# stripe/rainier

Measured on NVIDIA H100. Metric: leapfrog_steps_x_chains_per_sec, higher is better.
Workload: dtype f64

## Files before the change

rainier_b200/csrc/rn_runtime.cpp:

```cpp
#include <dlfcn.h>
#if defined(__x86_64__)
#include <emmintrin.h>
#endif
#include <nvrtc.h>
#include <sys/syscall.h>
#include <unistd.h>

#include <algorithm>
#include <atomic>
#include <cctype>
#include <chrono>
#include <cmath>
#include <cstdio>
#include <cstdlib>
#include <condition_variable>
#include <cstring>
#include <deque>
#include <functional>
#include <map>
#include <memory>
#include <mutex>
#include <sstream>
#include <string>
#include <thread>
// ... 131 lines not shown
}
static unsigned tpc_block_for(size_t chains, unsigned sms) {
  unsigned block = 128u;
  while (block > 32u && chains < (size_t)block * sms * 2) block >>= 1;
  if (const char* e = getenv("RN_BLOCK")) block = std::max(32u, std::min(128u, (unsigned)atoi(e) & ~31u));
  return block;
}
struct Kernel {
  std::string source;
  std::vector<char> cubin;
  CUmodule mod = nullptr;
  CUfunction k_init = nullptr, k_iter = nullptr, k_warmup = nullptr, k_density = nullptr, k_transpose = nullptr, k_pool_reduce = nullptr,
             k_pool_apply = nullptr, k_diag_chain = nullptr, k_diag_reduce = nullptr, k_step_pool = nullptr,
             k_diag_accum = nullptr, k_diag_terms = nullptr,
             k_pool_reduce_dense = nullptr, k_pool_factor = nullptr, k_pool_apply_dense = nullptr;
  const Program* prog = nullptr;
  int backend = 0;
  bool step_pool = false;
  bool mass_pool = false;
  unsigned tpc_block = 0;
  int wpc_smem_doubles = 0;
  int warps_per_cta = 4;
  int wpc_k = 1;
  int tma_stages = 0;
  int tile_doubles = 0;
  bool mma = false;
  int mma_chains = 8;
  unsigned tpc_smem_per_thread = 0;
  unsigned smem_bytes() const {
    size_t d = (size_t)warps_per_cta * wpc_smem_doubles;
    if (tma_stages > 0) d = ((d + 15) & ~(size_t)15) + (size_t)tma_stages * tile_doubles + (size_t)(mma ? 8 : tma_stages);
    return (unsigned)(d * 8);
  }
};

struct rn_model {
  std::recursive_mutex mu;
  std::vector<uint8_t> rir;
  uint32_t n_params = 0, n_inputs = 0;
  bool rir_has_gradient = false;
  int device = -1;
  CUcontext ctx = nullptr;
  CUdeviceptr d_data = 0;
  std::vector<uint64_t> target_base;
  std::vector<int> target_pitch;
  int inlined_targets = 0;
  int64_t inlined_monomials = 0, inlined_rows = 0;
  uint64_t data_doubles = 0;
  std::map<std::pair<bool, bool>, std::unique_ptr<Program>> programs;
  std::map<KernelKey, std::unique_ptr<Kernel>> kernels;
  CUdeviceptr pool[2] = {0, 0};
  CUdeviceptr diag_scratch = 0;
  size_t diag_bytes = 0;
  CUdeviceptr spare_arena = 0;
  size_t spare_arena_bytes = 0;
  CUstream spare_stream = nullptr;
  size_t pool_bytes[2] = {0, 0};
  struct OptKernel {
    std::string source;
    std::vector<char> cubin;
    CUmodule mod = nullptr;
    CUfunction k_lbfgs = nullptr;
    int backend = 0;
    int smem_doubles = 0;
    int starts_per_cta = 1;
    int wpc_k = 1;
  };
  std::map<std::tuple<bool, bool, int, int>, std::unique_ptr<OptKernel>> opt_kernels;
};

static int make_current(const Api* A, rn_model* m) {
  CU(A->cuCtxSetCurrent(m->ctx));
  return RN_OK;
}

static int get_program(rn_model* m, bool adjoint, bool fast, const Program** out) {
  if (!m->rir_has_gradient) adjoint = true;
  auto key = std::make_pair(adjoint, fast);
  auto it = m->programs.find(key);
  if (it == m->programs.end()) {
    std::unique_ptr<Program> P(new Program());
    std::string e = build_program(m->rir.data(), m->rir.size(), adjoint, fast, *P);
    if (!e.empty()) return fail(RN_E_INVALID, e);
    it = m->programs.emplace(key, std::move(P)).first;
  }
  *out = it->second.get();
  return RN_OK;
}

static KernelKey key_for(const rn_model* m, const rn_config* cfg) {
  KernelKey k;
  const int gm = cfg ? cfg->gradient_mode : RN_GRAD_AUTO;
  k.adjoint = (gm == RN_GRAD_ADJOINT) || !m->rir_has_gradient;
  k.fast = cfg && cfg->math_mode == RN_MATH_FAST;
  k.ehmc = cfg && cfg->sampler == RN_SAMPLER_EHMC;
  k.step_pool = cfg && cfg->step_adaptation == RN_ADAPT_POOLED;
  k.mass_pool = cfg && cfg->adaptation == RN_ADAPT_POOLED && cfg->mass_tuner == RN_MASS_DENSE;
  k.mass_max = 0;
  if (cfg) {
    if (cfg->mass_tuner == RN_MASS_DIAGONAL) k.mass_max = 1;
    if (cfg->mass_tuner == RN_MASS_DENSE) k.mass_max = 2;
    if (cfg->mass_tuner == RN_MASS_STATIC) k.mass_max = cfg->static_matrix == RN_MATRIX_DENSE ? 2 : (cfg->static_matrix == RN_MATRIX_DIAGONAL ? 1 : 0);
  }
  int want = cfg ? cfg->backend : RN_BACKEND_AUTO;
  if (const char* e = getenv("RN_BACKEND")) want = atoi(e);
  if (want == RN_BACKEND_AUTO) {
    uint64_t row_work = 0;
    auto it = m->programs.begin();
    if (it != m->programs.end())
      for (const TargetInfo& T : it->second->targets)
        if (T.streamed()) row_work += T.n_rows * (uint64_t)(T.row_fwd.size() + T.row_bwd.size() + 1);
    want = (row_work >= 16384 || m->n_params > 48) ? RN_BACKEND_WARP : RN_BACKEND_THREAD;
    if (k.mass_max == 2) want = RN_BACKEND_THREAD;
  }
  k.backend = want == RN_BACKEND_WARP ? 1 : 0;
  return k;
}

extern "C" const char* rn_version(void);
static int get_kernel(rn_model* m, const rn_config* cfg, Kernel** out, std::string* source_only = nullptr, size_t chains_hint = 0) {
  KernelKey key = key_for(m, cfg);
  if (key.backend == 0 && chains_hint > 0 && !(getenv("RN_GENERIC_BLOCK") && atoi(getenv("RN_GENERIC_BLOCK")) != 0)) key.block = (int)tpc_block_for(chains_hint, device_sms(m->device));
  auto it = m->kernels.find(key);
  if (it != m->kernels.end()) {
    if (source_only)
      *source_only = it->second->source;
    else
      *out = it->second.get();
    return RN_OK;
  }
  const Program* P = nullptr;
  int rc = get_program(m, key.adjoint, key.fast, &P);
  if (rc) return rc;
  std::unique_ptr<Kernel> K(new Kernel());
  K->prog = P;
  EmitOptions eo;
  eo.backend = key.backend;
  eo.fast_math = key.fast;
  eo.mass_max = key.mass_max;
  eo.enable_ehmc = key.ehmc;
  eo.step_pool = key.step_pool;
  eo.mass_pool = key.mass_pool;
  eo.target_base = m->target_base;
  eo.target_pitch = m->target_pitch;
  if (eo.backend == 1 && P->symbolic && P->n_params > 96)
    return fail(RN_E_UNSUPPORTED, "warp-per-chain with a symbolic gradient keeps n+1 accumulators in registers; use RN_GRAD_ADJOINT for n > 96");
  K->backend = eo.backend;
  K->step_pool = key.step_pool;
  K->mass_pool = key.mass_pool;
  K->tpc_block = (unsigned)key.block;
  if (eo.backend == 0) {
    const unsigned n = P->n_params;
    const unsigned doubles = (n + 1) + (key.mass_max >= 1 ? n : 0) + (key.ehmc ? n : 0) + 5 + 4;
    K->tpc_smem_per_thread = doubles * 8 + 10 * 4;
    if ((size_t)K->tpc_smem_per_thread * 32 > 227 * 1024 - 1024)
      return fail(RN_E_UNSUPPORTED, "thread-per-chain shape: the chain's shared-memory state does not fit; use RN_BACKEND_WARP");
  }
  if (eo.backend == 1) {
    const size_t cap = 227 * 1024 - 128;
    int wmax = 8;
    if (const char* e = getenv("RN_WPC_WARPS")) wmax = std::max(1, std::min(32, atoi(e)));
    {
      const WpcSizes z1 = wpc_sizes(*P, eo);
      const size_t pc = (size_t)z1.per_warp_doubles * 8;
      if (pc > cap) return fail(RN_E_UNSUPPORTED, "model state does not fit one chain's shared memory slice");
      const size_t fit = std::max<size_t>(1, (cap - std::min<size_t>(cap / 4, 2 * (size_t)z1.tile_doubles * 8)) / pc);
      int k = 1;
      while (k < 8 && fit * (size_t)k < 16) k *= 2;
      if (const char* e = getenv("RN_WPC_K")) k = std::max(1, std::min(8, atoi(e)));
      if (k != 1 && k != 2 && k != 4 && k != 8) k = 1;
      eo.wpc_k = K->wpc_k = k;
    }
    if (eo.wpc_k > 1) wmax = std::min(wmax, 14);
    const WpcSizes z = wpc_sizes(*P, eo);
    K->wpc_smem_doubles = z.per_warp_doubles;
    K->tile_doubles = z.tile_doubles;
    const size_t per_warp = (size_t)z.per_warp_doubles * 8, tile = (size_t)z.tile_doubles * 8;
    if (per_warp > cap) return fail(RN_E_UNSUPPORTED, "model state does not fit one chain's shared memory slice");
    int stages = 0;
    if (tile > 0) {
      if (2 * tile + std::min<size_t>(4, wmax) * per_warp + 256 <= cap)
        stages = 2;
      else if (tile + std::min<size_t>(2, wmax) * per_warp + 256 <= cap)
        stages = 1;
    }
    if (const char* e = getenv("RN_TMA")) {
      const int want_stages = atoi(e);
      if (want_stages == 0 || (size_t)want_stages * tile + per_warp + 256 <= cap) stages = tile > 0 ? want_stages : 0;
    }
    K->tma_stages = stages;
    const size_t left = cap - (size_t)stages * tile - (stages ? 256 : 0);
    K->warps_per_cta = (int)std::max<size_t>(1, std::min<size_t>((size_t)wmax, left / std::max<size_t>(per_warp, 1)));
    eo.tma_stages = stages;
    bool want_mma = !key.ehmc && key.mass_max < 2 && eo.wpc_k == 1 && z.mma_ok && !P->symbolic;
    if (const char* e = getenv("RN_MMA")) want_mma = want_mma && atoi(e) != 0;
    if (want_mma) {
      int want_chains = 16;
      if (const char* e = getenv("RN_MMA_CHAINS")) want_chains = atoi(e) >= 16 ? 16 : 8;
      for (int nc = want_chains; nc >= 8 && !K->mma; nc -= 8) {
        EmitOptions em = eo;
        em.mma = true;
        em.mma_chains = nc;
        em.tma_stages = 1;
        const WpcSizes zm = wpc_sizes(*P, em);
        const size_t need = (size_t)nc * (size_t)zm.per_warp_doubles * 8 + 128 + (size_t)zm.mma_shared_doubles * 8 + 64;
        if (zm.mma_ok && need <= cap) {
          eo = em;
          K->mma = true;
          K->mma_chains = nc;
          K->wpc_smem_doubles = zm.per_warp_doubles;
          K->tile_doubles = zm.mma_shared_doubles;
          K->tma_stages = 1;
          K->warps_per_cta = nc;
        }
      }
    }
  }
  if (eo.backend == 1) {
    const int warps = K->warps_per_cta * K->wpc_k;
    const int regs = warps * 32 * 255 > 65536 ? ((65536 / warps) / 512) * 512 / 32 : 255;
    int max_acc = 8;
    if (const char* e = getenv("RN_ROW_LIBM_MAX_ACC")) max_acc = atoi(e);
    const bool row_libm = getenv("RN_ROW_LIBM") ? atoi(getenv("RN_ROW_LIBM")) != 0 : (!eo.mma && wpc_sizes(*P, eo).reg_accumulators <= max_acc);
    eo.interleave = regs <= 128 ? (row_libm ? 2 : 4) : 8;
    if (const char* e = getenv("RN_INTERLEAVE")) eo.interleave = std::max(1, atoi(e));
  }
  K->source = emit_source(*P, eo);
  if (source_only) {
    *source_only = std::move(K->source);
    return RN_OK;
  }

  std::vector<const char*> opts = {"--gpu-architecture=sm_90a", "-std=c++17", "-lineinfo"};
  opts.push_back(key.fast ? "--fmad=true" : "--fmad=false");
  if (getenv("RN_LIBM_NOINLINE")) opts.push_back("-DRN_LIBM_NOINLINE=1");
  const std::string block_def = "-DRN_BLOCK_DIM=" + std::to_string(key.block);
  if (key.block > 0) opts.push_back(block_def.c_str());
  std::vector<std::string> extra_defs;
  if (const char* e = getenv("RN_NVRTC_DEFS")) {
    std::istringstream is(e);
    std::string tok;
    while (is >> tok) extra_defs.push_back(tok);
    for (const std::string& t : extra_defs) opts.push_back(t.c_str());
  }
  std::string maxreg;
  {
    int cap = (P->n_params <= 16 && eo.backend == 0) ? 128 : 0;
    if (eo.backend == 1) {
      const int warps = K->warps_per_cta * K->wpc_k;
      if (warps * 32 * 255 > 65536) cap = std::min(255, ((65536 / warps) / 512) * 512 / 32);
    }
    if (const char* e = getenv("RN_MAXRREGCOUNT")) cap = atoi(e);
    if (cap > 0) {
      maxreg = "--maxrregcount=" + std::to_string(cap);
      opts.push_back(maxreg.c_str());
    }
  }
  std::string cache_path;
  if (const char* dir = getenv("RN_KERNEL_CACHE")) {
    uint64_t h = 1469598103934665603ull;
    auto mix = [&](const std::string& t) {
      for (unsigned char ch : t) {
        h ^= ch;
        h *= 1099511628211ull;
      }
    };
    mix(K->source);
    for (const char* o : opts) mix(o);
    mix(rn_version());
    char name[64];
    snprintf(name, sizeof(name), "/%016llx.cubin", (unsigned long long)h);
    cache_path = std::string(dir) + name;
    if (FILE* f = fopen(cache_path.c_str(), "rb")) {
      fseek(f, 0, SEEK_END);
      long sz = ftell(f);
      fseek(f, 0, SEEK_SET);
      K->cubin.resize((size_t)sz);
      size_t got = fread(K->cubin.data(), 1, (size_t)sz, f);
      fclose(f);
      if (got == (size_t)sz && sz > 4) {
        *out = K.get();
        m->kernels.emplace(key, std::move(K));
        return RN_OK;
      }
      K->cubin.clear();
    }
  }
  nvrtcProgram prog;
  if (nvrtcCreateProgram(&prog, K->source.c_str(), "rainier_model.cu", 0, nullptr, nullptr) != NVRTC_SUCCESS)
    return fail(RN_E_COMPILE, "nvrtcCreateProgram failed");
  nvrtcResult r = nvrtcCompileProgram(prog, (int)opts.size(), opts.data());
  if (r != NVRTC_SUCCESS) {
    size_t n = 0;
    nvrtcGetProgramLogSize(prog, &n);
    std::string log(n, '\0');
    nvrtcGetProgramLog(prog, &log[0]);
    nvrtcDestroyProgram(&prog);
    if (const char* dump = getenv("RN_DUMP_FAILED_SOURCE")) {
      FILE* f = fopen(dump, "w");
      if (f) {
        fputs(K->source.c_str(), f);
        fclose(f);
      }
    }
    return fail(RN_E_COMPILE, std::string("NVRTC: ") + nvrtcGetErrorString(r) + "\n" + log);
  }
  size_t n = 0;
// ... 2449 lines not shown
```

rainier_b200/csrc/rn_sampler.cuh:

```cuda
#ifndef RN_SAMPLER_CUH
#define RN_SAMPLER_CUH


#if RN_MASS_MAX >= 1
#define RN_TS_NMASS RN_N
#else
#define RN_TS_NMASS 0
#endif
#if RN_ENABLE_EHMC
#define RN_TS_NSNAP RN_N
#else
#define RN_TS_NSNAP 0
#endif
#define RN_TS_P 0
#define RN_TS_MASS (RN_N + 1)
#define RN_TS_SNAP (RN_TS_MASS + RN_TS_NMASS)
#define RN_TS_STAT (RN_TS_SNAP + RN_TS_NSNAP)
#define RN_TS_HOT (RN_TS_STAT + 5)
#define RN_TS_DOUBLES (RN_TS_HOT + 4)
#define RN_TS_INTS 10
struct RnTs {
  double* d;
  int* i;
  unsigned bs;
};
#ifdef RN_HOST_EMULATION
static thread_local double rn_ts_mem_d[RN_TS_DOUBLES];
static thread_local int rn_ts_mem_i[RN_TS_INTS];
RN_DEVICE RnTs rn_ts_get() { return RnTs{rn_ts_mem_d, rn_ts_mem_i, 1u}; }
#define RN_STCS(ptr, v) (*(ptr) = (v))
#else
extern __shared__ double rn_ts_mem[];
RN_DEVICE RnTs rn_ts_get() {
  RnTs T;
#ifdef RN_BLOCK_DIM
  T.bs = RN_BLOCK_DIM;
#else
  T.bs = blockDim.x;
#endif
  T.d = rn_ts_mem + threadIdx.x;
  T.i = (int*)(rn_ts_mem + (size_t)RN_TS_DOUBLES * blockDim.x) + threadIdx.x;
  return T;
}
#define RN_STCS(ptr, v) __stcs((ptr), (v))
#endif
#define RN_TSD(slot) T.d[(unsigned)(slot) * T.bs]
#define RN_TSI(slot) T.i[(unsigned)(slot) * T.bs]
#ifndef RN_X_P_REGS
#define RN_X_P_REGS 1
#endif
#ifndef RN_X_NORMALS
#define RN_X_NORMALS 3
#endif
#define RN_Z(i) RN_TSD(RN_TS_P + (i))
#if RN_X_P_REGS
#define RN_P(i) s.p[i]
#else
#define RN_P(i) RN_TSD(RN_TS_P + (i))
#endif
#define RN_MASSD(i) RN_TSD(RN_TS_MASS + (i))
#define RN_SNAP_P(i) RN_TSD(RN_TS_SNAP + (i))
#define RN_ST_E_MEAN RN_TSD(RN_TS_STAT + 0)
#define RN_ST_E_RAW RN_TSD(RN_TS_STAT + 1)
#define RN_ST_TRANS2 RN_TSD(RN_TS_STAT + 2)
#define RN_ST_GRADS RN_TSD(RN_TS_STAT + 3)
#define RN_ST_STEPS RN_TSD(RN_TS_STAT + 4)
#define RN_ST_ITERS RN_TSI(0)
#define RN_ST_ACCEPTED RN_TSI(1)
#define RN_ST_E_N RN_TSI(2)
#define RN_ST_RING_I(r) RN_TSI(3 + (r))
#define RN_ST_RING_FULL(r) RN_TSI(6 + (r))
#define RN_TS_PREV_H RN_TSD(RN_TS_HOT + 2)
#define RN_TS_START_H RN_TSD(RN_TS_HOT + 3)

struct RnIt {
  int grads, steps, err;
};

RN_DEVICE RnRng rn_rng_unpark(const RnTs& T) {
  RnRng r;
  r.seed = rn_d2ll(RN_TSD(RN_TS_HOT + 0));
  r.nng = RN_TSD(RN_TS_HOT + 1);
  r.have = RN_TSI(9);
  return r;
}
RN_DEVICE void rn_rng_park(const RnTs& T, const RnRng& r) {
  RN_TSD(RN_TS_HOT + 0) = rn_ll2d(r.seed);
  RN_TSD(RN_TS_HOT + 1) = r.nng;
  RN_TSI(9) = r.have;
}

RN_DEVICE void rn_ring_add(const RnArgs& A, int c, const RnTs& T, int which, double value) {
  int i = RN_ST_RING_I(which) + 1;
  if (i == A.stats_window) {
    RN_ST_RING_FULL(which) = 1;
    i = 0;
  }
  RN_ST_RING_I(which) = i;
  RN_STCS(&RN_AT(A.st_rings, which * A.stats_window + i, c), value);
}

struct RnPQ {
  double q[RN_N], g[RN_N];
  double U;
#if RN_X_P_REGS
  double p[RN_N];
#endif
};

RN_DEVICE double rn_velocity_i(const RnArgs& A, int c, const RnTs& T, const RnPQ& s, int kind, int i) {
  (void)s;
  (void)T;
  (void)A;
  (void)c;
#if RN_MASS_MAX >= 2
  if (kind == 2) {
    double y = 0.0;
    for (int j = 0; j < RN_N; j++) y += RN_P(j) * RN_AT(A.mass, i * RN_N + j, c);
    return y;
  }
#endif
#if RN_MASS_MAX >= 1
  if (kind == 1) return RN_P(i) * RN_MASSD(i);
#endif
  (void)kind;
  return RN_P(i);
}

RN_DEVICE double rn_energy(const RnArgs& A, int c, const RnTs& T, const RnPQ& s, int kind, double U) {
  double k = 0.0;
#if RN_MASS_MAX >= 2
  if (kind == 2) {
    for (int i = 0; i < RN_N; i++) k += (rn_velocity_i(A, c, T, s, 2, i) * RN_P(i));
    return U + k / 2.0;
  }
#endif
  RN_UNROLL
  for (int i = 0; i < RN_N; i++) k += (rn_velocity_i(A, c, T, s, kind, i) * RN_P(i));
  return U + k / 2.0;
}

RN_DEVICE double rn_log_accept(double deltaH) {
  if (deltaH != deltaH) return -RN_INF;
  return rn_jmin0(-deltaH);
}


RN_DEVICE void rn_update(const RnArgs& A, RnPQ& s, RnIt& S) {
  double dens;
  rn_density(s.q, dens, s.g, A.data, S.err);
  s.U = dens * -1;
  S.grads += 1;
}
RN_DEVICE void rn_full_ps(const RnTs& T, RnPQ& s, double stepSize, RnIt& S) {
  (void)T;
  S.grads += 1;
  RN_UNROLL
  for (int i = 0; i < RN_N; i++) RN_P(i) += stepSize * s.g[i];
}
RN_DEVICE void rn_new_qs(const RnArgs& A, int c, const RnTs& T, int kind, RnPQ& s, double stepSize) {
#if RN_MASS_MAX >= 2
  if (kind == 2) {
    for (int i = 0; i < RN_N; i++) s.q[i] += (stepSize * rn_velocity_i(A, c, T, s, 2, i));
    return;
  }
#endif
  RN_UNROLL
  for (int i = 0; i < RN_N; i++) s.q[i] += (stepSize * rn_velocity_i(A, c, T, s, kind, i));
}
RN_DEVICE void rn_leapfrog(const RnArgs& A, int c, const RnTs& T, int kind, RnPQ& s, int l, double stepSize, RnIt& S) {
  rn_full_ps(T, s, stepSize / 2.0, S);
  for (int i = 0;;) {
    rn_new_qs(A, c, T, kind, s, stepSize);
    rn_update(A, s, S);
    if (++i >= l) break;
    rn_full_ps(T, s, stepSize, S);
  }
  rn_full_ps(T, s, stepSize / 2.0, S);
}
RN_DEVICE void rn_take_steps(const RnArgs& A, int c, const RnTs& T, int kind, RnPQ& s, int l, double stepSize, RnIt& S) {
  rn_ring_add(A, c, T, 0, stepSize);
  rn_leapfrog(A, c, T, kind, s, l, stepSize, S);
  S.steps += l;
}

RN_DEVICE void rn_draw_normals(const RnTs& T, RnRng& rng) {
#if RN_X_NORMALS == 2
  for (int i = 0; i < RN_N; i++) RN_Z(i) = rn_normal(rng);
  return;
#endif
  int i0 = 0;
  if (rng.have) {
    rng.have = 0;
    RN_Z(0) = rng.nng;
    i0 = 1;
  }
  const int npairs = (RN_N - i0 + 1) / 2;
#ifndef RN_X_POLAR2
#define RN_X_POLAR2 1
#endif
#if RN_X_POLAR2
  for (int k = 0; k < npairs;) {
    double a1, a2, b1, b2;
    rn_i64 seed4, seed8;
    rn_polar_attempt2(rng, a1, a2, b1, b2, seed4, seed8);
    const double sa = a1 * a1 + a2 * a2, sb = b1 * b1 + b2 * b2;
    const bool oka = !(sa >= 1 || sa == 0);
    const int kb = k + (oka ? 1 : 0);
    const bool needb = kb < npairs;
    const bool okb = needb && !(sb >= 1 || sb == 0);
    if (oka) {
      RN_Z(i0 + 2 * k) = a1;
      RN_Z(i0 + 2 * k + 1) = a2;
    }
    if (okb) {
      RN_Z(i0 + 2 * kb) = b1;
      RN_Z(i0 + 2 * kb + 1) = b2;
    }
    rng.seed = needb ? seed8 : seed4;
    k = kb + (okb ? 1 : 0);
  }
#else
  for (int k = 0; k < npairs;) {
    double v1, v2;
    rn_polar_attempt(rng, v1, v2);
    const double s = v1 * v1 + v2 * v2;
    if (!(s >= 1 || s == 0)) {
      RN_Z(i0 + 2 * k) = v1;
      RN_Z(i0 + 2 * k + 1) = v2;
      k += 1;
    }
  }
#endif
#if RN_X_NORMALS == 4 && RN_X_SPEC && !defined(RN_FAST_MATH) && !(defined(RN_X_LIBM_PLAIN) && RN_X_LIBM_PLAIN)
#pragma unroll 1
  for (int k = 0; k < npairs; k += 2) {
    const int ia = i0 + 2 * k, ib = i0 + 2 * (k + 1 < npairs ? k + 1 : k);
    const double a1 = RN_Z(ia), a2 = RN_Z(ia + 1), b1 = RN_Z(ib), b2 = RN_Z(ib + 1);
    const double sa = a1 * a1 + a2 * a2, sb = b1 * b1 + b2 * b2;
    bool oka, okb;
    double la = rn_strict_log_try(sa, oka), lb = rn_strict_log_try(sb, okb);
    if (!(oka && okb)) {
      la = rn_strict_log_full(sa);
      lb = rn_strict_log_full(sb);
    }
    const double ma = rn_sqrt_nc(rn_div_nc(-2 * la, sa)), mb = rn_sqrt_nc(rn_div_nc(-2 * lb, sb));
    RN_Z(ia) = a1 * ma;
    if (ia + 1 < RN_N) {
      RN_Z(ia + 1) = a2 * ma;
    } else {
      rng.nng = a2 * ma;
      rng.have = 1;
    }
    RN_Z(ib) = b1 * mb;
    if (ib + 1 < RN_N) {
      RN_Z(ib + 1) = b2 * mb;
    } else {
      rng.nng = b2 * mb;
      rng.have = 1;
    }
  }
  return;
#endif
#if RN_X_NORMALS == 1
#pragma unroll 1
#elif RN_X_NORMALS == 3
#pragma unroll 2
#endif
  for (int k = 0; k < npairs; k++) {
    const int i = i0 + 2 * k;
    const double v1 = RN_Z(i), v2 = RN_Z(i + 1);
    const double s = v1 * v1 + v2 * v2;
    const double multiplier = rn_polar_multiplier(s);
    RN_Z(i) = v1 * multiplier;
    if (i + 1 < RN_N) {
      RN_Z(i + 1) = v2 * multiplier;
    } else {
      rng.nng = v2 * multiplier;
      rng.have = 1;
    }
  }
}

RN_DEVICE void rn_initialize_ps(const RnArgs& A, int c, const RnTs& T, RnPQ& s, int kind, RnRng& rng) {
  (void)A;
  (void)c;
  (void)kind;
  (void)s;
  rn_draw_normals(T, rng);
#if RN_X_P_REGS
  RN_UNROLL
  for (int i = 0; i < RN_N; i++) s.p[i] = RN_Z(i);
#endif
#if RN_MASS_MAX >= 2
  if (kind == 2) {
    int i = RN_N - 1;
    int m = ((i + 1) * (i + 2)) / 2 - 1;
    while (i >= 0) {
      int j = RN_N - 1;
      double dot = 0.0;
      while (j > i) {
        dot += RN_Z(j) * RN_AT(A.chol, m, c);
        j -= 1;
        m -= 1;
      }
      RN_Z(i) = (RN_Z(i) - dot) / RN_AT(A.chol, m, c);
      i -= 1;
      m -= 1;
    }
#if RN_X_P_REGS
    for (int k = 0; k < RN_N; k++) s.p[k] = RN_Z(k);
#endif
    return;
  }
#endif
#if RN_MASS_MAX >= 1
  if (kind == 1) {
    RN_UNROLL
    for (int i = 0; i < RN_N; i++) RN_P(i) = RN_P(i) / sqrt(RN_MASSD(i));
    return;
  }
#endif
}

RN_DEVICE void rn_load_mass(const RnArgs& A, int c, const RnTs& T, int kind) {
  (void)A;
  (void)c;
  (void)T;
  (void)kind;
#if RN_MASS_MAX >= 1
  if (kind == 1) {
    RN_UNROLL
    for (int i = 0; i < RN_N; i++) RN_MASSD(i) = RN_AT(A.mass, i, c);
  }
#endif
}

RN_DEVICE void rn_load_stats(const RnArgs& A, int c, const RnTs& T) {
  RN_ST_GRADS = rn_ll2d(A.st_grads[c]);
  RN_ST_STEPS = rn_ll2d(A.st_steps[c]);
  RN_ST_ITERS = A.st_iters[c];
  RN_ST_ACCEPTED = A.st_accepted[c];
  RN_ST_E_MEAN = RN_AT(A.st_energy, 0, c);
  RN_ST_E_RAW = RN_AT(A.st_energy, 1, c);
  RN_ST_TRANS2 = RN_AT(A.st_energy, 2, c);
  RN_ST_E_N = A.st_energy_n[c];
  for (int r = 0; r < 3; r++) {
    RN_ST_RING_I(r) = RN_AT(A.st_ring_i, r, c);
    RN_ST_RING_FULL(r) = RN_AT(A.st_ring_full, r, c);
  }
}
RN_DEVICE void rn_store_stats(const RnArgs& A, int c, const RnTs& T, int err) {
  A.st_grads[c] = rn_d2ll(RN_ST_GRADS);
  A.st_steps[c] = rn_d2ll(RN_ST_STEPS);
  A.st_iters[c] = RN_ST_ITERS;
  A.st_accepted[c] = RN_ST_ACCEPTED;
  if (err) A.st_err[c] |= err;
  RN_AT(A.st_energy, 0, c) = RN_ST_E_MEAN;
  RN_AT(A.st_energy, 1, c) = RN_ST_E_RAW;
  RN_AT(A.st_energy, 2, c) = RN_ST_TRANS2;
  A.st_energy_n[c] = RN_ST_E_N;
  for (int r = 0; r < 3; r++) {
    RN_AT(A.st_ring_i, r, c) = RN_ST_RING_I(r);
    RN_AT(A.st_ring_full, r, c) = RN_ST_RING_FULL(r);
  }
}
RN_DEVICE void rn_fold(const RnTs& T, RnIt& S) {
  RN_ST_GRADS = rn_ll2d(rn_d2ll(RN_ST_GRADS) + (rn_i64)S.grads);
  RN_ST_STEPS = rn_ll2d(rn_d2ll(RN_ST_STEPS) + (rn_i64)S.steps);
  S.grads = 0;
  S.steps = 0;
}

RN_GLOBAL void rn_k_init(const RnArgs A) {
  const int c = (int)(blockIdx.x * blockDim.x + threadIdx.x);
  if (c >= A.chains) return;
  const RnTs T = rn_ts_get();
  RnRng rng;
  rng.seed = A.rng_seed[c];
  rng.nng = A.rng_nng[c];
  rng.have = A.rng_have[c];
  rn_load_stats(A, c, T);
  RnIt S;
  S.grads = 0;
  S.steps = 0;
  S.err = 0;

  RnPQ s;
  rn_draw_normals(T, rng);
  RN_UNROLL
  for (int i = 0; i < RN_N; i++) s.q[i] = RN_Z(i);
  rn_update(A, s, S);
  double cq[RN_N], cg[RN_N];
  const double cU = s.U;
  RN_UNROLL
  for (int i = 0; i < RN_N; i++) {
    cq[i] = s.q[i];
    cg[i] = s.g[i];
  }
  rn_initialize_ps(A, c, T, s, 0, rng);
  RN_UNROLL
  for (int i = 0; i < RN_N; i++) RN_AT(A.params, i, c) = RN_P(i);

  double stepSize;
  if (A.step_tuner == 0) {
    const double H0 = rn_energy(A, c, T, s, 0, cU);
    stepSize = 1.0;
    double lap;
    rn_leapfrog(A, c, T, 0, s, 1, stepSize, S);
    lap = rn_log_accept(rn_energy(A, c, T, s, 0, s.U) - H0);
    const double exponent = (lap > -RN_LN2) ? 1.0 : -1.0;
    const double doubleOrHalf = (exponent > 0) ? 2.0 : 0.5;
#if RN_STEP_POOL
    int log2Step = 0;
#endif
    while (stepSize != 0.0 && (exponent * lap > -exponent * RN_LN2)) {
      stepSize *= doubleOrHalf;
#if RN_STEP_POOL
      log2Step += (exponent > 0) ? 1 : -1;
#endif
      RN_UNROLL
      for (int i = 0; i < RN_N; i++) {
        RN_P(i) = RN_AT(A.params, i, c);
        s.q[i] = cq[i];
        s.g[i] = cg[i];
      }
      s.U = cU;
      rn_leapfrog(A, c, T, 0, s, 1, stepSize, S);
      lap = rn_log_accept(rn_energy(A, c, T, s, 0, s.U) - H0);
    }
    rn_da_apply(stepSize, RN_AT(A.da, 1, c), RN_AT(A.da, 2, c), RN_AT(A.da, 3, c), RN_AT(A.da, 4, c), A.da_iter[c]);
#if RN_STEP_POOL
    rn_pool_add_initial_step(A.step_acc, log2Step);
#endif
  } else {
    stepSize = A.static_step;
  }
  RN_AT(A.da, 0, c) = stepSize;

  RN_UNROLL
  for (int i = 0; i < RN_N; i++) {
    RN_AT(A.params, RN_N + i, c) = cq[i];
    RN_AT(A.grad, i, c) = cg[i];
  }
  RN_AT(A.params, 2 * RN_N, c) = cU;
  A.rng_seed[c] = rng.seed;
  A.rng_nng[c] = rng.nng;
  A.rng_have[c] = rng.have;
  rn_fold(T, S);
  rn_store_stats(A, c, T, S.err);
}

template <int PHASE>
RN_DEVICE void rn_iterate(const RnArgs& A) {
  const int c = A.chain_begin + (int)(blockIdx.x * blockDim.x + threadIdx.x);
  if (c >= A.chain_end) return;
  const RnTs T = rn_ts_get();
  {
    RnRng rng;
    rng.seed = A.rng_seed[c];
    rng.nng = A.rng_nng[c];
    rng.have = A.rng_have[c];
    rn_rng_park(T, rng);
  }
  rn_load_stats(A, c, T);
  RnIt S;
  S.grads = 0;
  S.steps = 0;
  S.err = 0;
  int kind = A.mass_kind;
  rn_load_mass(A, c, T, kind);

  double stepSize = RN_AT(A.da, 0, c);
  if (PHASE == 1 && A.step_tuner == 0) stepSize = rn_exp(RN_AT(A.da, 2, c));
  int win_size = A.win_size, win_i = A.win_i, win_j = A.win_j, est_samples = A.est_samples;
#if RN_ENABLE_EHMC
  int ring_i = 0, ring_full = 0;
  if (A.sampler == 1) {
    ring_i = A.ring_i[c];
    ring_full = A.ring_full[c];
  }
#endif
  bool havePrevH = false;

#ifndef RN_X_KEEP_STATE
#define RN_X_KEEP_STATE 1
#endif
#define RN_KEEP_P_LATE (RN_X_KEEP_STATE && RN_X_P_REGS)
  RnPQ s;
#if RN_X_KEEP_STATE
  RN_UNROLL
  for (int i = 0; i < RN_N; i++) {
    s.q[i] = RN_AT(A.params, RN_N + i, c);
    s.g[i] = RN_AT(A.grad, i, c);
  }
  s.U = RN_AT(A.params, 2 * RN_N, c);
#endif

  for (int it = 0; it < A.n_iter; it++) {
#if RN_X_KEEP_STATE
    const double cU = s.U;
#else
    const double cU = RN_AT(A.params, 2 * RN_N, c);
#endif
    if (!havePrevH) {
      RN_UNROLL
      for (int i = 0; i < RN_N; i++) RN_P(i) = RN_AT(A.params, i, c);
      RN_TS_PREV_H = rn_energy(A, c, T, s, kind, cU);
    }
    {
      RnRng rng = rn_rng_unpark(T);
      rn_initialize_ps(A, c, T, s, kind, rng);
      rn_rng_park(T, rng);
    }
#if RN_X_KEEP_STATE
    if (!(RN_KEEP_P_LATE && kind == 0)) {
      RN_UNROLL
      for (int i = 0; i < RN_N; i++) RN_AT(A.params, i, c) = RN_P(i);
    }
#else
    RN_UNROLL
    for (int i = 0; i < RN_N; i++) {
      RN_AT(A.params, i, c) = RN_P(i);
      s.q[i] = RN_AT(A.params, RN_N + i, c);
      s.g[i] = RN_AT(A.grad, i, c);
    }
#endif
    s.U = cU;
    RN_TS_START_H = rn_energy(A, c, T, s, kind, cU);
    const double usedStep = stepSize;

    if (A.sampler == 0) {
      rn_take_steps(A, c, T, kind, s, A.n_steps, stepSize, S);
    }
#if RN_ENABLE_EHMC
    else {
      bool count = false;
      if (PHASE == 0 && !ring_full) count = true;
      else if (PHASE == 0) {
        RnRng rng = rn_rng_unpark(T);
        count = rn_uniform(rng) < A.p_count;
        rn_rng_park(T, rng);
      }
      if (count) {
        RnPQ snap;
        int l = 0;
        for (;;) {
          double out = 0.0;
          RN_UNROLL
          for (int i = 0; i < RN_N; i++) out += (s.q[i] - RN_AT(A.params, RN_N + i, c)) * RN_P(i);
          const bool uturn = (out != out) ? true : (out < 0);
          if (uturn || !(l < A.max_steps)) break;
          l += 1;
          rn_take_steps(A, c, T, kind, s, 1, stepSize, S);
          if (l == A.min_steps) {
            snap = s;
#if !(RN_X_P_REGS)
            RN_UNROLL
            for (int i = 0; i < RN_N; i++) RN_SNAP_P(i) = RN_P(i);
#endif
          }
        }
        if (l < A.min_steps) {
          rn_take_steps(A, c, T, kind, s, A.min_steps - l, stepSize, S);
        } else {
          s = snap;
#if !(RN_X_P_REGS)
          RN_UNROLL
          for (int i = 0; i < RN_N; i++) RN_P(i) = RN_SNAP_P(i);
#endif
        }
        ring_i += 1;
        if (ring_i == A.buf_size) ring_full = 1;
        ring_i = ring_i % A.buf_size;
        RN_AT(A.ring, ring_i, c) = (double)l;
      } else {
        RnRng rng = rn_rng_unpark(T);
        const int idx = ring_full ? rn_rng_int(rng, A.buf_size) : rn_rng_int(rng, ring_i + 1);
        rn_rng_park(T, rng);
        const int nsteps = rn_d2i(RN_AT(A.ring, idx, c));
        rn_take_steps(A, c, T, kind, s, nsteps, stepSize, S);
      }
    }
#endif

    const double endH = rn_energy(A, c, T, s, kind, s.U);
    const double startH = RN_TS_START_H;
    const double deltaH = endH - startH;
    const double a = rn_log_accept(deltaH);
    bool accept;
    {
      RnRng rng = rn_rng_unpark(T);
      accept = a > rn_log(rn_uniform(rng));
      rn_rng_park(T, rng);
    }
    double eH;
    if (accept) {
      RN_UNROLL
      for (int i = 0; i < RN_N; i++) {
        RN_AT(A.params, i, c) = RN_P(i);
        RN_AT(A.params, RN_N + i, c) = s.q[i];
        RN_AT(A.grad, i, c) = s.g[i];
      }
      RN_AT(A.params, 2 * RN_N, c) = s.U;
      eH = endH;
      RN_ST_ACCEPTED += 1;
    } else {
      RN_UNROLL
      for (int i = 0; i < RN_N; i++) s.q[i] = RN_AT(A.params, RN_N + i, c);
#if RN_X_KEEP_STATE
      RN_UNROLL
      for (int i = 0; i < RN_N; i++) s.g[i] = RN_AT(A.grad, i, c);
      s.U = RN_AT(A.params, 2 * RN_N, c);
      if (RN_KEEP_P_LATE && kind == 0) {
        RN_UNROLL
        for (int i = 0; i < RN_N; i++) RN_AT(A.params, i, c) = RN_Z(i);
      }
#endif
      eH = startH;
    }
    {
      const int e_n = RN_ST_E_N + 1;
      RN_ST_E_N = e_n;
      double e_mean = RN_ST_E_MEAN;
      const double oldDiff = eH - e_mean;
      e_mean += (oldDiff / (double)e_n);
      RN_ST_E_MEAN = e_mean;
      const double newDiff = eH - e_mean;
      RN_ST_E_RAW += oldDiff * newDiff;
      const double d = eH - RN_TS_PREV_H;
      RN_ST_TRANS2 += d * d;
    }
    RN_TS_PREV_H = eH;
    havePrevH = true;
    RN_ST_ITERS += 1;
    rn_ring_add(A, c, T, 1, rn_exp(a));
    rn_ring_add(A, c, T, 2, (double)S.grads);

    if (A.trace) {
      double* tr = A.trace + (size_t)it * 4 * (size_t)A.chains;
      tr[0 * (size_t)A.chains + c] = a;
      tr[1 * (size_t)A.chains + c] = accept ? 1.0 : 0.0;
      tr[2 * (size_t)A.chains + c] = usedStep;
      tr[3 * (size_t)A.chains + c] = (double)S.steps;
    }
    rn_fold(T, S);

    if (PHASE == 0) {
#if RN_STEP_POOL
      if (A.step_tuner == 0) rn_pool_add(A.step_acc + it, rn_pool_quantise(rn_exp(a)));
#else
      if (A.step_tuner == 0) {
        const double newAcceptanceProb = rn_exp(a);
        const int daIter = A.da_iter[c] + 1;
        A.da_iter[c] = daIter;
        const double avgErrorMultiplier = 1.0 / ((double)daIter + 10);
        const double stepSizeMultiplier = rn_pow((double)daIter, -0.75);
        const double avgError = ((1.0 - avgErrorMultiplier) * RN_AT(A.da, 3, c) + (avgErrorMultiplier * (A.delta - newAcceptanceProb)));
        RN_AT(A.da, 3, c) = avgError;
        const double logStepSize = (RN_AT(A.da, 4, c) - (avgError * sqrt((double)daIter) / 0.05));
        RN_AT(A.da, 1, c) = logStepSize;
        RN_AT(A.da, 2, c) = (stepSizeMultiplier * logStepSize + (1.0 - stepSizeMultiplier) * RN_AT(A.da, 2, c));
        stepSize = rn_exp(logStepSize);
      }
#endif
#if RN_MASS_MAX >= 1
      if (A.mass_tuner == 1 || A.mass_tuner == 2) {
        win_j += 1;
        if (A.adaptation == 1) {
          if (RN_IN_WINDOW(A, win_j)) {
            win_i += 1;
#if RN_MASS_POOL
            double oldDiff[RN_N], newDiff[RN_N];
            RN_UNROLL
            for (int i = 0; i < RN_N; i++) newDiff[i] = rn_variance_update(A, c, i, s.q[i], win_i, oldDiff[i]);
            for (int j = 0; j < RN_N; j++)
              for (int k = 0; k < RN_N; k++) RN_AT(A.est_cov, j * RN_N + k, c) += newDiff[j] * oldDiff[k];
#else
            RN_UNROLL
            for (int i = 0; i < RN_N; i++) {
              double oldDiff;
              rn_variance_update(A, c, i, s.q[i], win_i, oldDiff);
            }
#endif
            if (win_i == win_size) {
              win_i = 0;
              win_size = rn_d2i(win_size * A.win_expansion);
            }
          }
        } else if (RN_IN_WINDOW(A, win_j)) {
          win_i += 1;
          est_samples += 1;
#if RN_MASS_MAX >= 2
          double oldDiff[RN_N], newDiff[RN_N];
          RN_UNROLL
          for (int i = 0; i < RN_N; i++) newDiff[i] = rn_variance_update(A, c, i, s.q[i], est_samples, oldDiff[i]);
#else
          RN_UNROLL
          for (int i = 0; i < RN_N; i++) {
            double oldDiff;
            rn_variance_update(A, c, i, s.q[i], est_samples, oldDiff);
          }
#endif
#if RN_MASS_MAX >= 2
          if (A.mass_tuner == 2) {
            for (int j = 0; j < RN_N; j++)
              for (int k = 0; k < RN_N; k++) RN_AT(A.est_cov, j * RN_N + k, c) += newDiff[j] * oldDiff[k];
          }
#endif
          if (win_i == win_size) {
            win_i = 0;
            win_size = rn_d2i(win_size * A.win_expansion);
            havePrevH = false;
            if (A.mass_tuner == 1) {
              kind = 1;
              RN_UNROLL
              for (int i = 0; i < RN_N; i++) {
                const double v = RN_AT(A.est_raw, i, c) / (double)est_samples;
                if (v == 0.0) S.err |= 2;
                RN_MASSD(i) = v;
                RN_AT(A.mass, i, c) = v;
                RN_AT(A.est_mean, i, c) = 0.0;
                RN_AT(A.est_raw, i, c) = 0.0;
              }
            }
#if RN_MASS_MAX >= 2
            else {
              kind = 2;
              const double z = (double)(est_samples - 1);
              for (int i = 0; i < RN_N * RN_N; i++) {
                const double v = RN_AT(A.est_cov, i, c) / z;
                if (v == 0.0) S.err |= 2;
                RN_AT(A.mass, i, c) = v;
                RN_AT(A.est_cov, i, c) = 0.0;
              }
              for (int i = 0; i < RN_N; i++) {
                RN_AT(A.est_mean, i, c) = 0.0;
                RN_AT(A.est_raw, i, c) = 0.0;
              }
              double lower[(RN_N * (RN_N + 1)) / 2];
              rn_cholesky_upper(A, c, lower, 1);
            }
#endif
#if !RN_STEP_POOL
            if (A.step_tuner == 0)
              stepSize = rn_da_reset(RN_AT(A.da, 1, c), RN_AT(A.da, 2, c), RN_AT(A.da, 3, c), RN_AT(A.da, 4, c), A.da_iter[c]);
#endif
          }
        }
      }
#endif
    } else if (A.samples) {
      double* out = A.samples + (size_t)it * RN_N * (size_t)A.chains;
      RN_UNROLL
      for (int i = 0; i < RN_N; i++) RN_STCS(&out[(size_t)i * (size_t)A.chains + c], s.q[i]);
    }
  }

  if (PHASE == 0) RN_AT(A.da, 0, c) = stepSize;
#if RN_ENABLE_EHMC
  if (A.sampler == 1) {
    A.ring_i[c] = ring_i;
    A.ring_full[c] = ring_full;
  }
#endif
  {
    const RnRng rng = rn_rng_unpark(T);
    A.rng_seed[c] = rng.seed;
    A.rng_nng[c] = rng.nng;
    A.rng_have[c] = rng.have;
  }
  rn_store_stats(A, c, T, S.err);
}
// ... 25 lines not shown
```

Measured before the change: 25.06 billion.

## Add pipelined next-iteration normal draws inside leapfrog and pinned address computation for accept writes

Adds an optional path (RN_X_PIPE_DRAWS, off by default) that generates the next iteration's momentum normals incrementally between leapfrog steps, storing them in an extra shared-memory region, so RNG latency overlaps with gradient work. It also pre-draws the accept uniform. It enables by default an inline-asm trick (rn_site) that pins the per-chain params/grad base pointers and stride, so the accept/reject stores use simple strided addressing. The host always reserves extra shared memory per thread for the pipeline buffer, which may lower occupancy or reject shapes that used to fit.

Result: faster. 27.00 billion (median of 6 runs) (+7.7%).

```diff
diff --git a/rainier_b200/csrc/rn_runtime.cpp b/rainier_b200/csrc/rn_runtime.cpp
--- a/rainier_b200/csrc/rn_runtime.cpp
+++ b/rainier_b200/csrc/rn_runtime.cpp
@@ -307,7 +307,7 @@
   if (eo.backend == 0) {
     const unsigned n = P->n_params;
     const unsigned doubles = (n + 1) + (key.mass_max >= 1 ? n : 0) + (key.ehmc ? n : 0) + 5 + 4;
-    K->tpc_smem_per_thread = doubles * 8 + 10 * 4;
+    K->tpc_smem_per_thread = doubles * 8 + 10 * 4 + (n + 1) * 8;
     if ((size_t)K->tpc_smem_per_thread * 32 > 227 * 1024 - 1024)
       return fail(RN_E_UNSUPPORTED, "thread-per-chain shape: the chain's shared-memory state does not fit; use RN_BACKEND_WARP");
   }
diff --git a/rainier_b200/csrc/rn_sampler.cuh b/rainier_b200/csrc/rn_sampler.cuh
--- a/rainier_b200/csrc/rn_sampler.cuh
+++ b/rainier_b200/csrc/rn_sampler.cuh
@@ -19,13 +19,24 @@
 #define RN_TS_HOT (RN_TS_STAT + 5)
 #define RN_TS_DOUBLES (RN_TS_HOT + 4)
 #define RN_TS_INTS 10
+#ifndef RN_X_PIPE_DRAWS
+#define RN_X_PIPE_DRAWS 0
+#endif
+#ifndef RN_X_PIPE_QUOTA
+#define RN_X_PIPE_QUOTA 2
+#endif
+#define RN_TS_ZN (RN_TS_DOUBLES + RN_TS_INTS / 2)
 struct RnTs {
   double* d;
   int* i;
   unsigned bs;
 };
 #ifdef RN_HOST_EMULATION
+#if RN_X_PIPE_DRAWS
+static thread_local double rn_ts_mem_d[RN_TS_ZN + RN_N + 1];
+#else
 static thread_local double rn_ts_mem_d[RN_TS_DOUBLES];
+#endif
 static thread_local int rn_ts_mem_i[RN_TS_INTS];
 RN_DEVICE RnTs rn_ts_get() { return RnTs{rn_ts_mem_d, rn_ts_mem_i, 1u}; }
 #define RN_STCS(ptr, v) (*(ptr) = (v))
@@ -43,6 +54,23 @@
   return T;
 }
 #define RN_STCS(ptr, v) __stcs((ptr), (v))
+#endif
+#ifndef RN_X_SITE_ADDR
+#define RN_X_SITE_ADDR 1
+#endif
+#if RN_X_SITE_ADDR
+#ifdef RN_HOST_EMULATION
+template <class V> RN_DEVICE V rn_site(V v) { return v; }
+#else
+RN_DEVICE double* rn_site(double* p) {
+  asm volatile("mov.b64 %0, %0;" : "+l"(p));
+  return p;
+}
+RN_DEVICE size_t rn_site(size_t v) {
+  asm volatile("mov.b64 %0, %0;" : "+l"(v));
+  return v;
+}
+#endif
 #endif
 #define RN_TSD(slot) T.d[(unsigned)(slot) * T.bs]
 #define RN_TSI(slot) T.i[(unsigned)(slot) * T.bs]
@@ -168,39 +196,41 @@
   RN_UNROLL
   for (int i = 0; i < RN_N; i++) s.q[i] += (stepSize * rn_velocity_i(A, c, T, s, kind, i));
 }
-RN_DEVICE void rn_leapfrog(const RnArgs& A, int c, const RnTs& T, int kind, RnPQ& s, int l, double stepSize, RnIt& S) {
+struct RnPipe;
+#if RN_X_PIPE_DRAWS
+RN_DEVICE void rn_pipe_step(const RnTs& T, RnPipe& P);
+#endif
+template <int PIPE = 0>
+RN_DEVICE void rn_leapfrog(const RnArgs& A, int c, const RnTs& T, int kind, RnPQ& s, int l, double stepSize, RnIt& S,
+                           RnPipe* P = nullptr) {
   rn_full_ps(T, s, stepSize / 2.0, S);
   for (int i = 0;;) {
     rn_new_qs(A, c, T, kind, s, stepSize);
+#if RN_X_PIPE_DRAWS
+    if constexpr (PIPE != 0) rn_pipe_step(T, *P);
+#endif
     rn_update(A, s, S);
     if (++i >= l) break;
     rn_full_ps(T, s, stepSize, S);
   }
   rn_full_ps(T, s, stepSize / 2.0, S);
 }
-RN_DEVICE void rn_take_steps(const RnArgs& A, int c, const RnTs& T, int kind, RnPQ& s, int l, double stepSize, RnIt& S) {
+template <int PIPE = 0>
+RN_DEVICE void rn_take_steps(const RnArgs& A, int c, const RnTs& T, int kind, RnPQ& s, int l, double stepSize, RnIt& S,
+                             RnPipe* P = nullptr) {
   rn_ring_add(A, c, T, 0, stepSize);
-  rn_leapfrog(A, c, T, kind, s, l, stepSize, S);
+  rn_leapfrog<PIPE>(A, c, T, kind, s, l, stepSize, S, P);
   S.steps += l;
 }
 
-RN_DEVICE void rn_draw_normals(const RnTs& T, RnRng& rng) {
-#if RN_X_NORMALS == 2
-  for (int i = 0; i < RN_N; i++) RN_Z(i) = rn_normal(rng);
-  return;
-#endif
-  int i0 = 0;
-  if (rng.have) {
-    rng.have = 0;
-    RN_Z(0) = rng.nng;
-    i0 = 1;
-  }
+#define RN_ZB(i) RN_TSD(zb + (i))
+RN_DEVICE void rn_normals_from(const RnTs& T, RnRng& rng, unsigned zb, int i0, int k0, int m0) {
   const int npairs = (RN_N - i0 + 1) / 2;
 #ifndef RN_X_POLAR2
 #define RN_X_POLAR2 1
 #endif
 #if RN_X_POLAR2
-  for (int k = 0; k < npairs;) {
+  for (int k = k0; k < npairs;) {
     double a1, a2, b1, b2;
     rn_i64 seed4, seed8;
     rn_polar_attempt2(rng, a1, a2, b1, b2, seed4, seed8);
@@ -210,33 +240,33 @@
     const bool needb = kb < npairs;
     const bool okb = needb && !(sb >= 1 || sb == 0);
     if (oka) {
-      RN_Z(i0 + 2 * k) = a1;
-      RN_Z(i0 + 2 * k + 1) = a2;
+      RN_ZB(i0 + 2 * k) = a1;
+      RN_ZB(i0 + 2 * k + 1) = a2;
     }
     if (okb) {
-      RN_Z(i0 + 2 * kb) = b1;
-      RN_Z(i0 + 2 * kb + 1) = b2;
+      RN_ZB(i0 + 2 * kb) = b1;
+      RN_ZB(i0 + 2 * kb + 1) = b2;
     }
     rng.seed = needb ? seed8 : seed4;
     k = kb + (okb ? 1 : 0);
   }
 #else
-  for (int k = 0; k < npairs;) {
+  for (int k = k0; k < npairs;) {
     double v1, v2;
     rn_polar_attempt(rng, v1, v2);
     const double s = v1 * v1 + v2 * v2;
     if (!(s >= 1 || s == 0)) {
-      RN_Z(i0 + 2 * k) = v1;
-      RN_Z(i0 + 2 * k + 1) = v2;
+      RN_ZB(i0 + 2 * k) = v1;
+      RN_ZB(i0 + 2 * k + 1) = v2;
       k += 1;
     }
   }
 #endif
 #if RN_X_NORMALS == 4 && RN_X_SPEC && !defined(RN_FAST_MATH) && !(defined(RN_X_LIBM_PLAIN) && RN_X_LIBM_PLAIN)
 #pragma unroll 1
-  for (int k = 0; k < npairs; k += 2) {
+  for (int k = m0; k < npairs; k += 2) {
     const int ia = i0 + 2 * k, ib = i0 + 2 * (k + 1 < npairs ? k + 1 : k);
-    const double a1 = RN_Z(ia), a2 = RN_Z(ia + 1), b1 = RN_Z(ib), b2 = RN_Z(ib + 1);
+    const double a1 = RN_ZB(ia), a2 = RN_ZB(ia + 1), b1 = RN_ZB(ib), b2 = RN_ZB(ib + 1);
     const double sa = a1 * a1 + a2 * a2, sb = b1 * b1 + b2 * b2;
     bool oka, okb;
     double la = rn_strict_log_try(sa, oka), lb = rn_strict_log_try(sb, okb);
@@ -245,16 +275,16 @@
       lb = rn_strict_log_full(sb);
     }
     const double ma = rn_sqrt_nc(rn_div_nc(-2 * la, sa)), mb = rn_sqrt_nc(rn_div_nc(-2 * lb, sb));
-    RN_Z(ia) = a1 * ma;
+    RN_ZB(ia) = a1 * ma;
     if (ia + 1 < RN_N) {
-      RN_Z(ia + 1) = a2 * ma;
+      RN_ZB(ia + 1) = a2 * ma;
     } else {
       rng.nng = a2 * ma;
       rng.have = 1;
     }
-    RN_Z(ib) = b1 * mb;
+    RN_ZB(ib) = b1 * mb;
     if (ib + 1 < RN_N) {
-      RN_Z(ib + 1) = b2 * mb;
+      RN_ZB(ib + 1) = b2 * mb;
     } else {
       rng.nng = b2 * mb;
       rng.have = 1;
@@ -267,27 +297,125 @@
 #elif RN_X_NORMALS == 3
 #pragma unroll 2
 #endif
-  for (int k = 0; k < npairs; k++) {
+  for (int k = m0; k < npairs; k++) {
     const int i = i0 + 2 * k;
-    const double v1 = RN_Z(i), v2 = RN_Z(i + 1);
+    const double v1 = RN_ZB(i), v2 = RN_ZB(i + 1);
     const double s = v1 * v1 + v2 * v2;
     const double multiplier = rn_polar_multiplier(s);
-    RN_Z(i) = v1 * multiplier;
+    RN_ZB(i) = v1 * multiplier;
     if (i + 1 < RN_N) {
-      RN_Z(i + 1) = v2 * multiplier;
+      RN_ZB(i + 1) = v2 * multiplier;
     } else {
       rng.nng = v2 * multiplier;
       rng.have = 1;
     }
   }
 }
-
-RN_DEVICE void rn_initialize_ps(const RnArgs& A, int c, const RnTs& T, RnPQ& s, int kind, RnRng& rng) {
+RN_DEVICE void rn_draw_normals(const RnTs& T, RnRng& rng) {
+#if RN_X_NORMALS == 2
+  for (int i = 0; i < RN_N; i++) RN_Z(i) = rn_normal(rng);
+  return;
+#endif
+  int i0 = 0;
+  if (rng.have) {
+    rng.have = 0;
+    RN_Z(0) = rng.nng;
+    i0 = 1;
+  }
+  rn_normals_from(T, rng, RN_TS_P, i0, 0, 0);
+}
+
+#if RN_X_PIPE_DRAWS
+struct RnPipe {
+  rn_i64 seed;
+  int i0;
+  int k;
+  int m;
+};
+#define RN_ZN(i) RN_TSD(RN_TS_ZN + (i))
+RN_DEVICE RnPipe rn_pipe_start(const RnTs& T, const RnRng& rng) {
+  RnPipe P;
+  P.seed = rng.seed;
+  P.i0 = rng.have;
+  P.k = 0;
+  P.m = 0;
+  if (rng.have) RN_ZN(0) = rng.nng;
+  return P;
+}
+RN_DEVICE void rn_pipe_trip(const RnTs& T, RnPipe& P) {
+  const int npairs = (RN_N - P.i0 + 1) / 2;
+  RnRng r;
+  r.seed = P.seed;
+  double a1, a2, b1, b2;
+  rn_i64 seed4, seed8;
+  rn_polar_attempt2(r, a1, a2, b1, b2, seed4, seed8);
+  const double sa = a1 * a1 + a2 * a2, sb = b1 * b1 + b2 * b2;
+  const bool need = P.k < npairs;
+  const bool oka = need && !(sa >= 1 || sa == 0);
+  const int kb = P.k + (oka ? 1 : 0);
+  const bool needb = kb < npairs;
+  const bool okb = needb && !(sb >= 1 || sb == 0);
+  const int ia = P.i0 + 2 * P.k, ib = P.i0 + 2 * kb;
+  if (oka) {
+    RN_ZN(ia) = a1;
+    RN_ZN(ia + 1) = a2;
+  }
+  if (okb) {
+    RN_ZN(ib) = b1;
+    RN_ZN(ib + 1) = b2;
+  }
+  P.seed = need ? (needb ? seed8 : seed4) : P.seed;
+  P.k = kb + (okb ? 1 : 0);
+}
+RN_DEVICE void rn_pipe_mult(const RnTs& T, RnPipe& P) {
+#if !defined(RN_FAST_MATH) && RN_X_SPEC && !(defined(RN_X_LIBM_PLAIN) && RN_X_LIBM_PLAIN)
+  const bool ready = P.m < P.k;
+  const int i = ready ? P.i0 + 2 * P.m : 0;
+  const double v1 = RN_ZN(i), v2 = RN_ZN(i + 1);
+  const double s = ready ? v1 * v1 + v2 * v2 : 0.5;
+  bool ok;
+  const double l = rn_strict_log_try(s, ok);
+  const double mult = rn_sqrt_nc(rn_div_nc(-2 * l, s));
+  if (ready && ok) {
+    RN_ZN(i) = v1 * mult;
+    RN_ZN(i + 1) = v2 * mult;
+    P.m += 1;
+  }
+#else
+  (void)T;
+  (void)P;
+#endif
+}
+RN_DEVICE void rn_pipe_step(const RnTs& T, RnPipe& P) {
+#if RN_X_PIPE_QUOTA
+#if RN_X_PIPE_QUOTA >= 2
+  rn_pipe_mult(T, P);
+#endif
+  rn_pipe_trip(T, P);
+#else
+  (void)T;
+  (void)P;
+#endif
+}
+RN_DEVICE void rn_pipe_finish(const RnTs& T, const RnPipe& P, RnRng& rng) {
+  const unsigned zb = RN_TS_ZN;
+  const int npairs = (RN_N - P.i0 + 1) / 2;
+  const bool lastDone = P.m == npairs;
+  rng.seed = P.seed;
+  rng.have = 0;
+  rn_normals_from(T, rng, zb, P.i0, P.k, P.m);
+  if (lastDone && ((RN_N - P.i0) & 1)) {
+    rng.nng = RN_ZB(RN_N);
+    rng.have = 1;
+  }
+}
+#endif
+
+RN_DEVICE void rn_momentum_from_z(const RnArgs& A, int c, const RnTs& T, RnPQ& s, int kind) {
   (void)A;
   (void)c;
   (void)kind;
   (void)s;
-  rn_draw_normals(T, rng);
 #if RN_X_P_REGS
   RN_UNROLL
   for (int i = 0; i < RN_N; i++) s.p[i] = RN_Z(i);
@@ -322,6 +450,10 @@
   }
 #endif
 }
+RN_DEVICE void rn_initialize_ps(const RnArgs& A, int c, const RnTs& T, RnPQ& s, int kind, RnRng& rng) {
+  rn_draw_normals(T, rng);
+  rn_momentum_from_z(A, c, T, s, kind);
+}
 
 RN_DEVICE void rn_load_mass(const RnArgs& A, int c, const RnTs& T, int kind) {
   (void)A;
@@ -496,6 +628,10 @@
   }
   s.U = RN_AT(A.params, 2 * RN_N, c);
 #endif
+#if RN_X_PIPE_DRAWS
+  const bool pipe = !RN_ENABLE_EHMC || A.sampler == 0;
+  bool pipeFull = false;
+#endif
 
   for (int it = 0; it < A.n_iter; it++) {
 #if RN_X_KEEP_STATE
@@ -510,7 +646,19 @@
     }
     {
       RnRng rng = rn_rng_unpark(T);
-      rn_initialize_ps(A, c, T, s, kind, rng);
+#if RN_X_PIPE_DRAWS
+      if (pipe) {
+        if (pipeFull) {
+          RN_UNROLL
+          for (int i = 0; i < RN_N; i++) RN_Z(i) = RN_ZN(i);
+        } else {
+          rn_draw_normals(T, rng);
+        }
+        rn_momentum_from_z(A, c, T, s, kind);
+        RN_Z(RN_N) = rn_uniform(rng);
+      } else
+#endif
+        rn_initialize_ps(A, c, T, s, kind, rng);
       rn_rng_park(T, rng);
     }
 #if RN_X_KEEP_STATE
@@ -531,7 +679,18 @@
     const double usedStep = stepSize;
 
     if (A.sampler == 0) {
+#if RN_X_PIPE_DRAWS
+      RnPipe P = rn_pipe_start(T, rn_rng_unpark(T));
+      rn_take_steps<1>(A, c, T, kind, s, A.n_steps, stepSize, S, &P);
+      if (it + 1 < A.n_iter) {
+        RnRng rng = rn_rng_unpark(T);
+        rn_pipe_finish(T, P, rng);
+        rn_rng_park(T, rng);
+        pipeFull = true;
+      }
+#else
       rn_take_steps(A, c, T, kind, s, A.n_steps, stepSize, S);
+#endif
     }
 #if RN_ENABLE_EHMC
     else {
@@ -589,36 +748,53 @@
     const double deltaH = endH - startH;
     const double a = rn_log_accept(deltaH);
     bool accept;
+#if RN_X_PIPE_DRAWS
+    if (pipe) {
+      accept = a > rn_log(RN_Z(RN_N));
+    } else
+#endif
     {
       RnRng rng = rn_rng_unpark(T);
       accept = a > rn_log(rn_uniform(rng));
       rn_rng_park(T, rng);
     }
     double eH;
+#if RN_X_SITE_ADDR
+    double* const pa = rn_site(A.params + c);
+    double* const ga = rn_site(A.grad + c);
+    const size_t cs = rn_site((size_t)A.chains);
+#define RN_PA(field) pa[(size_t)(field) * cs]
+#define RN_GA(field) ga[(size_t)(field) * cs]
+#else
+#define RN_PA(field) RN_AT(A.params, field, c)
+#define RN_GA(field) RN_AT(A.grad, field, c)
+#endif
     if (accept) {
       RN_UNROLL
       for (int i = 0; i < RN_N; i++) {
-        RN_AT(A.params, i, c) = RN_P(i);
-        RN_AT(A.params, RN_N + i, c) = s.q[i];
-        RN_AT(A.grad, i, c) = s.g[i];
+        RN_PA(i) = RN_P(i);
+        RN_PA(RN_N + i) = s.q[i];
+        RN_GA(i) = s.g[i];
       }
-      RN_AT(A.params, 2 * RN_N, c) = s.U;
+      RN_PA(2 * RN_N) = s.U;
       eH = endH;
       RN_ST_ACCEPTED += 1;
     } else {
       RN_UNROLL
-      for (int i = 0; i < RN_N; i++) s.q[i] = RN_AT(A.params, RN_N + i, c);
+      for (int i = 0; i < RN_N; i++) s.q[i] = RN_PA(RN_N + i);
 #if RN_X_KEEP_STATE
       RN_UNROLL
-      for (int i = 0; i < RN_N; i++) s.g[i] = RN_AT(A.grad, i, c);
-      s.U = RN_AT(A.params, 2 * RN_N, c);
+      for (int i = 0; i < RN_N; i++) s.g[i] = RN_GA(i);
+      s.U = RN_PA(2 * RN_N);
       if (RN_KEEP_P_LATE && kind == 0) {
         RN_UNROLL
-        for (int i = 0; i < RN_N; i++) RN_AT(A.params, i, c) = RN_Z(i);
+        for (int i = 0; i < RN_N; i++) RN_PA(i) = RN_Z(i);
       }
 #endif
       eH = startH;
     }
+#undef RN_PA
+#undef RN_GA
     {
       const int e_n = RN_ST_E_N + 1;
       RN_ST_E_N = e_n;
```
